# Ghostish/Open3DSOT

Hardware: AMD Instinct MI355X
Metric: template/search pairs/sec (fwd+bwd), BAT KITTI-Car 512/1024 pts (higher is better)
Workload: dtype f32; 1 GPU; BAT_Car.yaml KITTI-Car, template 512 / search 1024 pts, batch 48 per GPU, fwd+bwd+Adam, fp32; global_batch=48, parallelism=dp1, fused_kernels=True, hip_graph=True, rccl_world_size=1

## Files before the change

### open3dsot_amd/csrc/mlp_direct.hip

```cpp
#include <type_traits>
#include "mlp_common.hpp"

namespace {

constexpr int DT_M = 64;

template <int NT>
__device__ __forceinline__ void ldv(float (&d)[NT], const float* p) {
    if constexpr (NT == 4) {
        const float4 t = *reinterpret_cast<const float4*>(p);
        d[0] = t.x; d[1] = t.y; d[2] = t.z; d[3] = t.w;
    } else if constexpr (NT == 2) {
        const float2 t = *reinterpret_cast<const float2*>(p);
        d[0] = t.x; d[1] = t.y;
    } else {
        d[0] = *p;
    }
}
template <int NT>
__device__ __forceinline__ void stv(float* p, const float (&d)[NT]) {
    if constexpr (NT == 4)      *reinterpret_cast<float4*>(p) = make_float4(d[0], d[1], d[2], d[3]);
    else if constexpr (NT == 2) *reinterpret_cast<float2*>(p) = make_float2(d[0], d[1]);
    else                        *p = d[0];
}

template <int NT>
struct RawB {
    float v[4][NT];
    float y[4][NT];
    float4 c1, c2, c3;
};

enum BMode { B_PLAIN = 0, B_XFORM = 1, B_DY = 2, B_DYPOOL = 3 };

struct DirectArgs {
    const float* A;
    const float* X;
    const float* Y;
    const float* c1; const float* c2; const float* c3;
    const float2* pk; int ns;
    float* Out;
    int M, K, P, B;
    const float* w;
    const int32_t* meta;
    long start1;
    float* part;
    const float* stat_c;
    const float* Yprev; const float* scale_p; const float* shift_p; const float* mean_p;
    const float* bias;
    const float* resid;
    const float* cbias; int cb_N, cb_B;
    int tail_slots; long extra_row0;
};

template <int MODE, int NT>
__device__ __forceinline__ void load_b(const DirectArgs& a, const float* xb, const float* yb, long rowP, int kb,
                                       long pool_base, int np, RawB<NT>& f) {
#pragma unroll
    for (int s = 0; s < 4; ++s) {
        if (MODE != B_DYPOOL) ldv<NT>(f.v[s], xb + (long)(kb + s) * rowP);
        if (MODE >= B_DY) ldv<NT>(f.y[s], yb + (long)(kb + s) * rowP);
        if constexpr (MODE == B_DYPOOL && NT >= 2) {
            const float2 t = a.pk[pool_base + (long)(kb + s) * np];
            f.v[s][0] = t.x; f.v[s][1] = t.y;
        }
    }
    if (MODE != B_PLAIN) {
        f.c1 = *reinterpret_cast<const float4*>(a.c1 + kb);
        f.c2 = *reinterpret_cast<const float4*>(a.c2 + kb);
        if (MODE >= B_DY) f.c3 = *reinterpret_cast<const float4*>(a.c3 + kb);
    }
}

template <int MODE, int NT, int MT>
__device__ __forceinline__ void compute_group(const RawB<NT>& f, const float4& a0v, const float4& a1v, int kk,
                                              const float (&wv)[NT], f32x16 (&acc)[MT][NT]) {
    const float a0[4] = {a0v.x, a0v.y, a0v.z, a0v.w}, a1[4] = {a1v.x, a1v.y, a1v.z, a1v.w};
    const float c1[4] = {f.c1.x, f.c1.y, f.c1.z, f.c1.w}, c2[4] = {f.c2.x, f.c2.y, f.c2.z, f.c2.w};
    const float c3[4] = {f.c3.x, f.c3.y, f.c3.z, f.c3.w};
#pragma unroll
    for (int s = 0; s < 4; ++s) {
        float bv[NT];
        if constexpr (MODE == B_DYPOOL && NT >= 2) {
            const float go = f.v[s][0];
            const int ak = __float_as_int(f.v[s][1]);
#pragma unroll
            for (int t = 0; t < NT; ++t) bv[t] = (kk + t == ak) ? go : 0.f;
        } else {
#pragma unroll
            for (int t = 0; t < NT; ++t) bv[t] = f.v[s][t];
        }
        if (MODE == B_XFORM) {
#pragma unroll
            for (int t = 0; t < NT; ++t) bv[t] = fmaxf(fmaf(bv[t], c1[s], c2[s]), 0.f);
        } else if (MODE >= B_DY) {
#pragma unroll
            for (int t = 0; t < NT; ++t) bv[t] = fmaf(c1[s], bv[t], wv[t] * fmaf(c2[s], f.y[s][t], c3[s]));
        }
#pragma unroll
        for (int t = 0; t < NT; ++t) {
            acc[0][t] = mfma32(a0[s], bv[t], acc[0][t]);
            if constexpr (MT == 2) acc[1][t] = mfma32(a1[s], bv[t], acc[1][t]);
        }
    }
}

template <int WAVES, int MODE, int EPI, int NT, int MT = 2>
__device__ __forceinline__ void direct_gemm_body(DirectArgs& a, const int bx, const int by, const long part_row = -1) {
    constexpr int POS = 32 * NT;
    constexpr int DT_MW = 32 * MT;
    const int lane = threadIdx.x & 63, wave = threadIdx.x >> 6;
    const int l31 = lane & 31, h = lane >> 5;
    const int tiles_per_b = a.P / POS;
    const int tile = bx;
    const int b = tile / tiles_per_b, p0 = (tile - b * tiles_per_b) * POS;
    if (a.meta) {
        const long c0 = (long)tile * POS;
        const int seg = (a.start1 > 0 && c0 >= a.start1) ? 1 : 0;
        if (c0 - (seg ? a.start1 : 0) >= a.meta[4 * seg]) return;
        if (seg) {
            if (a.c1) a.c1 += a.K;
            if (a.c2) a.c2 += a.K;
            if (a.c3) a.c3 += a.K;
            if (a.stat_c) a.stat_c += a.M;
            if (a.scale_p) { a.scale_p += a.M; a.shift_p += a.M; a.mean_p += a.M; }
        }
    }
    const int m0 = (by * WAVES + wave) * DT_MW;
    const int p = p0 + NT * l31;
    float wv[NT];
#pragma unroll
    for (int t = 0; t < NT; ++t) wv[t] = 1.f;
    if (a.w) ldv<NT>(wv, a.w + (long)b * a.P + p);
    const long rowP = a.P;
    const float* xb = (MODE != B_DYPOOL) ? a.X + (long)b * a.K * rowP + p : nullptr;
    const float* yb = (MODE >= B_DY) ? a.Y + (long)b * a.K * rowP + p : nullptr;
    const float* wa = a.A + (long)(m0 + l31) * a.K + 4 * h;
    const long wstep = 32L * a.K;
    int np = 1, kk = 0;
    long pool_base = 0;
    if (MODE == B_DYPOOL) {
        np = a.P / a.ns;
        const int j = p / a.ns;
        kk = p - j * a.ns;
        pool_base = (long)b * a.K * np + j;
    }

    f32x16 acc[MT][NT];
#pragma unroll
    for (int i = 0; i < MT; ++i)
#pragma unroll
        for (int t = 0; t < NT; ++t)
#pragma unroll
            for (int r = 0; r < 16; ++r) acc[i][t][r] = 0.f;

    const int G = a.K / 8;
    RawB<NT> f[2];
    float4 wa0[2], wa1[2];
    auto load = [&](auto stc, int g) {
        constexpr int st = decltype(stc)::value;
        const int kb = 8 * g + 4 * h;
        load_b<MODE, NT>(a, xb, yb, rowP, kb, pool_base, np, f[st]);
        wa0[st] = *reinterpret_cast<const float4*>(wa + 8 * g);
        if constexpr (MT == 2) wa1[st] = *reinterpret_cast<const float4*>(wa + 8 * g + wstep);
        else wa1[st] = wa0[st];
    };
    {
        load(std::integral_constant<int, 0>{}, 0);
        for (int g = 0; g < G; g += 2) {
            load(std::integral_constant<int, 1>{}, g + 1);
            __builtin_amdgcn_sched_barrier(0);
            compute_group<MODE, NT, MT>(f[0], wa0[0], wa1[0], kk, wv, acc);
            __builtin_amdgcn_sched_barrier(0);
            load(std::integral_constant<int, 0>{}, g + 2 < G ? g + 2 : G - 1);
            __builtin_amdgcn_sched_barrier(0);
            compute_group<MODE, NT, MT>(f[1], wa0[1], wa1[1], kk, wv, acc);
            __builtin_amdgcn_sched_barrier(0);
        }
    }

    int cloud = 0;
    if constexpr (EPI == 3) cloud = (int)(((long)b * a.P + p0) / a.cb_N);
    const bool stats = EPI != 2 && a.part != nullptr;
    float4 kc1[MT][4], kc2[MT][4];
    if constexpr (EPI != 1) {
#pragma unroll
        for (int i = 0; i < MT; ++i)
#pragma unroll
            for (int q = 0; q < 4; ++q) {
                const int mb = m0 + 32 * i + 4 * h + 8 * q;
                kc1[i][q] = kc2[i][q] = make_float4(0.f, 0.f, 0.f, 0.f);
                if constexpr (EPI == 2) {
                    if (a.bias) kc1[i][q] = *reinterpret_cast<const float4*>(a.bias + mb);
                } else {
                    if (a.stat_c) kc1[i][q] = *reinterpret_cast<const float4*>(a.stat_c + mb);
                    if constexpr (EPI == 3) {
                        kc2[i][q].x = a.cbias[(long)(mb + 0) * a.cb_B + cloud];
                        kc2[i][q].y = a.cbias[(long)(mb + 1) * a.cb_B + cloud];
                        kc2[i][q].z = a.cbias[(long)(mb + 2) * a.cb_B + cloud];
                        kc2[i][q].w = a.cbias[(long)(mb + 3) * a.cb_B + cloud];
                    }
                }
            }
    }
#pragma unroll
    for (int i = 0; i < MT; ++i) {
        float red[32];
#pragma unroll
        for (int hb = 0; hb < 2; ++hb) {
            const int mb = m0 + 32 * i + 16 * hb + 4 * h;
            const long ob = ((long)b * a.M + mb) * rowP + p;
            float ex[8][NT];
            float4 k1[2], k2[2], k3[2];
            if constexpr (EPI == 1 || EPI == 2) {
                const float* src = EPI == 1 ? a.Yprev : a.resid;
#pragma unroll
                for (int r = 0; r < 8; ++r) {
#pragma unroll
                    for (int t = 0; t < NT; ++t) ex[r][t] = 0.f;
                    if (EPI == 1 || src) ldv<NT>(ex[r], src + ob + (long)(8 * (r >> 2) + (r & 3)) * rowP);
                }
            }
#pragma unroll
            for (int q = 0; q < 2; ++q) {
                k3[q] = make_float4(0.f, 0.f, 0.f, 0.f);
                if constexpr (EPI == 1) {
                    k1[q] = *reinterpret_cast<const float4*>(a.scale_p + mb + 8 * q);
                    k2[q] = *reinterpret_cast<const float4*>(a.shift_p + mb + 8 * q);
                    k3[q] = *reinterpret_cast<const float4*>(a.mean_p + mb + 8 * q);
                } else {
                    k1[q] = kc1[i][2 * hb + q];
                    k2[q] = kc2[i][2 * hb + q];
                }
            }
#pragma unroll
            for (int r8 = 0; r8 < 8; ++r8) {
                const int q = r8 >> 2, j = r8 & 3, r = 8 * hb + r8;
                const float c1 = j == 0 ? k1[q].x : j == 1 ? k1[q].y : j == 2 ? k1[q].z : k1[q].w;
                const float c2 = j == 0 ? k2[q].x : j == 1 ? k2[q].y : j == 2 ? k2[q].z : k2[q].w;
                const float c3 = j == 0 ? k3[q].x : j == 1 ? k3[q].y : j == 2 ? k3[q].z : k3[q].w;
                float v[NT];
#pragma unroll
                for (int t = 0; t < NT; ++t) v[t] = acc[i][t][r];
                float s1 = 0.f, s2 = 0.f;
                if constexpr (EPI == 1) {
#pragma unroll
                    for (int t = 0; t < NT; ++t) {
                        v[t] = fmaf(ex[r8][t], c1, c2) > 0.f ? v[t] : 0.f;
                        s1 += v[t];
                        s2 = fmaf(v[t], ex[r8][t] - c3, s2);
                    }
                } else if constexpr (EPI == 2) {
#pragma unroll
                    for (int t = 0; t < NT; ++t) v[t] = (v[t] + c1) + ex[r8][t];
                } else {
#pragma unroll
                    for (int t = 0; t < NT; ++t) {
                        if constexpr (EPI == 3) v[t] += c2;
                        s1 = fmaf(wv[t], v[t], s1);
                        s2 += wv[t] * (v[t] - c1) * (v[t] - c1);
                    }
                }
                stv<NT>(a.Out + ob + (long)(8 * q + j) * rowP, v);
                red[r] = s1;
                red[16 + r] = s2;
            }
        }
        if (stats) {
            reduce_scatter32(red, l31);
            a.part[(part_row >= 0 ? part_row : (long)tile) * 2 * a.M + (long)(l31 >> 4) * a.M + m0 + 32 * i + acc_row(l31 & 15, h)] = red[0];
        }
    }
}


template <int WAVES, int MODE, int EPI, int NT, int MT = 2>
__global__ __launch_bounds__(WAVES * 64) __attribute__((amdgpu_waves_per_eu(2, (NT == 4 && MT == 2) ? 2 : 4)))
void direct_gemm_kernel(DirectArgs a) {
    direct_gemm_body<WAVES, MODE, EPI, NT, MT>(a, blockIdx.x, blockIdx.y);
}

template <int WAVES, int MODE, int EPI>
__global__ __launch_bounds__(WAVES * 64) __attribute__((amdgpu_waves_per_eu(2, 2)))
void direct_gemm_tail_kernel(DirectArgs a) {
    const int tile = blockIdx.x;
    const int seg = (a.start1 > 0 && (long)tile * 128 >= a.start1) ? 1 : 0;
    const int t0 = seg ? (int)(a.start1 / 128) : 0;
    const int cap = a.start1 > 0 ? (seg ? (int)((a.P - a.start1) / 128) : (int)(a.start1 / 128)) : a.P / 128;
    const int T = a.meta[4 * seg] / 128;
    const TailPlan pl = tail_plan(T, a.tail_slots, cap);
    const int tl = tile - t0;
    if (tl < pl.full) { direct_gemm_body<WAVES, MODE, EPI, 4, 2>(a, tile, blockIdx.y); return; }
    const int u = tl - pl.full;
    if (u >= pl.R * pl.f) return;
    const int j = u / pl.f, blk = u - j * pl.f;
    const int tt = t0 + pl.full + j;
    const long row = blk == 0 ? (long)tt : a.extra_row0 + (long)seg * a.tail_slots + (long)j * (pl.f - 1) + (blk - 1);
    if (pl.f == 4) direct_gemm_body<WAVES, MODE, EPI, 1, 2>(a, tt * 4 + blk, blockIdx.y, row);
    else           direct_gemm_body<WAVES, MODE, EPI, 2, 2>(a, tt * 2 + blk, blockIdx.y, row);
}

template <int WAVES, int MODE, int EPI, int NT, int MT>
__global__ __launch_bounds__(WAVES * 64) __attribute__((amdgpu_waves_per_eu(2, NT == 4 ? 2 : 4)))
void direct_gemm_pair_kernel(DirectArgs a0, DirectArgs a1) {
    if (blockIdx.z == 0) {
        if ((int)blockIdx.y * WAVES * 32 * MT < a0.M) direct_gemm_body<WAVES, MODE, EPI, NT, MT>(a0, blockIdx.x, blockIdx.y);
    } else {
        if ((int)blockIdx.y * WAVES * 32 * MT < a1.M) direct_gemm_body<WAVES, MODE, EPI, NT, MT>(a1, blockIdx.x, blockIdx.y);
    }
}

constexpr int SK_ROWS = 32, SK_COLS = 64;

__device__ __forceinline__ float reduce_scatter8(float (&x)[8], int l31) {
#pragma unroll
    for (int m = 4; m >= 1; m >>= 1) {
        const bool up = (l31 & m) != 0;
#pragma unroll
        for (int v = 0; v < m; ++v) {
            float lo = x[v], hi = x[v + m];
            asm volatile("" : "+v"(lo), "+v"(hi));
            const float keep = up ? hi : lo;
            const float send = up ? lo : hi;
            x[v] = keep + __shfl_xor(send, m, 64);
        }
    }
    float r = x[0];
    r += __shfl_xor(r, 8, 64);
    r += __shfl_xor(r, 16, 64);
    return r;
}

template <int MODE, int EPI>
__device__ __forceinline__ void splitk_body(DirectArgs& a, const int bx, const int by, float* __restrict__ red) {
    static_assert(MODE <= B_DY && EPI <= 2, "split-K tile: plain / transformed / BatchNorm-backward operands only");
    constexpr int NT = 2;
    const int lane = threadIdx.x & 63, wave = threadIdx.x >> 6;
    const int l31 = lane & 31, h = lane >> 5;
    const int tiles_per_b = a.P / SK_COLS;
    const int tile = bx;
    const int b = tile / tiles_per_b, p0 = (tile - b * tiles_per_b) * SK_COLS;
    if (a.meta) {
        const long c0 = (long)tile * SK_COLS;
        const int seg = (a.start1 > 0 && c0 >= a.start1) ? 1 : 0;
        if (c0 - (seg ? a.start1 : 0) >= a.meta[4 * seg]) return;
        if (seg) {
            if (a.c1) a.c1 += a.K;
            if (a.c2) a.c2 += a.K;
            if (a.c3) a.c3 += a.K;
            if (a.stat_c) a.stat_c += a.M;
            if (a.scale_p) { a.scale_p += a.M; a.shift_p += a.M; a.mean_p += a.M; }
        }
    }
    const int m0 = by * SK_ROWS;
    const int p = p0 + NT * l31;
    float wv[NT] = {1.f, 1.f};
    if (a.w) ldv<NT>(wv, a.w + (long)b * a.P + p);
    const long rowP = a.P;
    const float* xb = a.X + (long)b * a.K * rowP + p;
    const float* yb = (MODE >= B_DY) ? a.Y + (long)b * a.K * rowP + p : nullptr;
    const float* wa = a.A + (long)(m0 + l31) * a.K + 4 * h;

    const int mrow = m0 + 8 * wave + 4 * h;
    const long ob = ((long)b * a.M + mrow) * rowP + p;
    float ex[4][NT];
    float4 k1 = make_float4(0.f, 0.f, 0.f, 0.f), k2 = k1, k3 = k1;
    if constexpr (EPI == 1 || EPI == 2) {
        const float* src = EPI == 1 ? a.Yprev : a.resid;
#pragma unroll
        for (int j = 0; j < 4; ++j) {
            ex[j][0] = ex[j][1] = 0.f;
            if (EPI == 1 || src) ldv<NT>(ex[j], src + ob + (long)j * rowP);
        }
    }
    if constexpr (EPI == 1) {
        k1 = *reinterpret_cast<const float4*>(a.scale_p + mrow);
        k2 = *reinterpret_cast<const float4*>(a.shift_p + mrow);
        k3 = *reinterpret_cast<const float4*>(a.mean_p + mrow);
    } else if constexpr (EPI == 2) {
        if (a.bias) k1 = *reinterpret_cast<const float4*>(a.bias + mrow);
    } else {
        if (a.stat_c) k1 = *reinterpret_cast<const float4*>(a.stat_c + mrow);
    }

    f32x16 acc[1][NT];
#pragma unroll
    for (int t = 0; t < NT; ++t)
#pragma unroll
        for (int r = 0; r < 16; ++r) acc[0][t][r] = 0.f;

    const int npair = a.K / 16;
    const int q = npair / 4, rem = npair - 4 * q;
    const int ps = wave * q + (wave < rem ? wave : rem);
    const int gs = 2 * ps, ge = 2 * (ps + q + (wave < rem ? 1 : 0));
    RawB<NT> f[2];
    float4 wa0[2];
    auto load = [&](auto stc, int g) {
        constexpr int st = decltype(stc)::value;
        load_b<MODE, NT>(a, xb, yb, rowP, 8 * g + 4 * h, 0, 1, f[st]);
        wa0[st] = *reinterpret_cast<const float4*>(wa + 8 * g);
    };
    if (gs < ge) {
        load(std::integral_constant<int, 0>{}, gs);
        for (int g = gs; g < ge; g += 2) {
            load(std::integral_constant<int, 1>{}, g + 1);
            __builtin_amdgcn_sched_barrier(0);
            compute_group<MODE, NT, 1>(f[0], wa0[0], wa0[0], 0, wv, acc);
            __builtin_amdgcn_sched_barrier(0);
            load(std::integral_constant<int, 0>{}, g + 2 < ge ? g + 2 : ge - 1);
            __builtin_amdgcn_sched_barrier(0);
            compute_group<MODE, NT, 1>(f[1], wa0[1], wa0[1], 0, wv, acc);
            __builtin_amdgcn_sched_barrier(0);
        }
    }

#pragma unroll
    for (int r = 0; r < 16; ++r)
        *reinterpret_cast<float2*>(red + ((wave * SK_ROWS + acc_row(r, h)) * SK_COLS + NT * l31)) =
            make_float2(acc[0][0][r], acc[0][1][r]);
    __syncthreads();
    float x8[8];
    const bool stats = EPI != 2 && a.part != nullptr;
#pragma unroll
    for (int j = 0; j < 4; ++j) {
        const int row = 8 * wave + 4 * h + j;
        float v[NT] = {0.f, 0.f};
#pragma unroll
        for (int w4 = 0; w4 < 4; ++w4) {
            const float2 t = *reinterpret_cast<const float2*>(red + ((w4 * SK_ROWS + row) * SK_COLS + NT * l31));
            v[0] += t.x; v[1] += t.y;
        }
        const float c1 = j == 0 ? k1.x : j == 1 ? k1.y : j == 2 ? k1.z : k1.w;
        const float c2 = j == 0 ? k2.x : j == 1 ? k2.y : j == 2 ? k2.z : k2.w;
        const float c3 = j == 0 ? k3.x : j == 1 ? k3.y : j == 2 ? k3.z : k3.w;
        float s1 = 0.f, s2 = 0.f;
        if constexpr (EPI == 1) {
#pragma unroll
            for (int t = 0; t < NT; ++t) {
                v[t] = fmaf(ex[j][t], c1, c2) > 0.f ? v[t] : 0.f;
                s1 += v[t];
                s2 = fmaf(v[t], ex[j][t] - c3, s2);
            }
        } else if constexpr (EPI == 2) {
#pragma unroll
            for (int t = 0; t < NT; ++t) v[t] = (v[t] + c1) + ex[j][t];
        } else {
#pragma unroll
            for (int t = 0; t < NT; ++t) {
                s1 = fmaf(wv[t], v[t], s1);
                s2 += wv[t] * (v[t] - c1) * (v[t] - c1);
            }
        }
        stv<NT>(a.Out + ob + (long)j * rowP, v);
        x8[j] = s1;
        x8[4 + j] = s2;
    }
    if (stats) {
        const float r = reduce_scatter8(x8, l31);
        if (l31 < 8) a.part[(long)tile * 2 * a.M + (long)(l31 >> 2) * a.M + mrow + (l31 & 3)] = r;
    }
}

template <int MODE, int EPI>
__global__ __launch_bounds__(256) __attribute__((amdgpu_waves_per_eu(3, 4)))
void splitk_gemm_kernel(DirectArgs a) {
    __shared__ float red[4 * SK_ROWS * SK_COLS];
    splitk_body<MODE, EPI>(a, blockIdx.x, blockIdx.y, red);
}

template <int MODE, int EPI>
__global__ __launch_bounds__(256) __attribute__((amdgpu_waves_per_eu(3, 4)))
void splitk_gemm_pair_kernel(DirectArgs a0, DirectArgs a1) {
    __shared__ float red[4 * SK_ROWS * SK_COLS];
    if (blockIdx.z == 0) {
        if ((int)blockIdx.y * SK_ROWS < a0.M) splitk_body<MODE, EPI>(a0, blockIdx.x, blockIdx.y, red);
    } else {
        if ((int)blockIdx.y * SK_ROWS < a1.M) splitk_body<MODE, EPI>(a1, blockIdx.x, blockIdx.y, red);
    }
}

static long splitk_max() { return 16L << 20; }
static bool splitk_ok(const DirectArgs& a, int tile) {
    return tile == 64 && a.K % 16 == 0 && a.K >= 64 && a.M % SK_ROWS == 0 && a.P % SK_COLS == 0 && !a.pk &&
           (long)a.M * a.B * a.P <= splitk_max();
}
template <int MODE, int EPI>
int launch_splitk(const DirectArgs& a, hipStream_t st) {
    if constexpr (MODE <= B_DY && EPI <= 2) {
        hipLaunchKernelGGL((splitk_gemm_kernel<MODE, EPI>), dim3(a.B * (a.P / SK_COLS), a.M / SK_ROWS), dim3(256), 0, st, a);
        return o3d_launch_status();
    } else {
        return O3D_EINVAL;
    }
}

template <int MODE, int EPI, int NT, int MT = 2>
int launch_direct_nt(const DirectArgs& a, hipStream_t st) {
    const int tiles = a.B * (a.P / (32 * NT));
    const int slabs = a.M / (32 * MT);
    if constexpr (NT == 4 && MT == 2 && MODE != B_DYPOOL && EPI <= 1) {
        if (a.tail_slots > 0 && a.meta && a.B == 1) {
            if (slabs % 4 == 0)      hipLaunchKernelGGL((direct_gemm_tail_kernel<4, MODE, EPI>), dim3(tiles, slabs / 4), dim3(256), 0, st, a);
            else if (slabs % 2 == 0) hipLaunchKernelGGL((direct_gemm_tail_kernel<2, MODE, EPI>), dim3(tiles, slabs / 2), dim3(128), 0, st, a);
            else                     hipLaunchKernelGGL((direct_gemm_tail_kernel<1, MODE, EPI>), dim3(tiles, slabs), dim3(64), 0, st, a);
            return o3d_launch_status();
        }
    }
    if (slabs % 4 == 0) {
        hipLaunchKernelGGL((direct_gemm_kernel<4, MODE, EPI, NT, MT>), dim3(tiles, slabs / 4), dim3(256), 0, st, a);
    } else if (slabs % 2 == 0) {
        hipLaunchKernelGGL((direct_gemm_kernel<2, MODE, EPI, NT, MT>), dim3(tiles, slabs / 2), dim3(128), 0, st, a);
    } else {
        hipLaunchKernelGGL((direct_gemm_kernel<1, MODE, EPI, NT, MT>), dim3(tiles, slabs), dim3(64), 0, st, a);
    }
    return o3d_launch_status();
}

static int pw_tile(long P, int M) { return o3d_direct_tile(P, M, 0); }

template <int MODE, int EPI>
int launch_direct_small(const DirectArgs& a, int tile, hipStream_t st) {
    if constexpr (MODE <= B_DY && EPI <= 2) {
        if (splitk_ok(a, tile)) return launch_splitk<MODE, EPI>(a, st);
    }
    if constexpr (MODE != B_DYPOOL) {
        if (tile == 128 && a.M <= 128) return launch_direct_nt<MODE, EPI, 4, 1>(a, st);
    }
    return tile == 64 ? launch_direct_nt<MODE, EPI, 2>(a, st) : launch_direct_nt<MODE, EPI, 4>(a, st);
}

template <int MODE, int EPI>
int launch_direct(const DirectArgs& a, int tile, hipStream_t st) {
    if constexpr (MODE <= B_DY && EPI <= 2) {
        if (splitk_ok(a, tile)) return launch_splitk<MODE, EPI>(a, st);
    }
    return tile == 64 ? launch_direct_nt<MODE, EPI, 2>(a, st) : launch_direct_nt<MODE, EPI, 4>(a, st);
}

}

bool o3d_direct_ok(int M, int K, int P) { return M % DT_M == 0 && K % 16 == 0 && P % 128 == 0; }

static int g_tail_override = -1;
extern "C" int o3d_direct_tail_override(int slots) { g_tail_override = slots; return O3D_OK; }

extern "C" int o3d_direct_tail_slots(int M) {
    if (g_tail_override >= 0) return (M > 0 && M % DT_M == 0) ? g_tail_override : 0;
    static int cus_of[64] = {};
    int dev = 0;
    if (hipGetDevice(&dev) != hipSuccess || dev < 0 || dev >= 64) dev = 0;
    if (cus_of[dev] == 0) {
        int n = 0;
        if (hipDeviceGetAttribute(&n, hipDeviceAttributeMultiprocessorCount, dev) != hipSuccess || n <= 0) n = 256;
        cus_of[dev] = n;
    }
    const int cus = cus_of[dev];
    if (M <= 0 || M % DT_M != 0) return 0;
    const int slabs = M / DT_M;
    const int waves = slabs % 4 == 0 ? 4 : (slabs % 2 == 0 ? 2 : 1);
    const int per_tile = slabs / waves;
    const int slots = (8 / waves) * cus / per_tile;
    return slots >= 64 ? slots : 0;
}

extern "C" int o3d_direct_tile(long P, int M, int compact) {
    (void)M; (void)compact;
    return P <= 65536L ? 64 : 128;
}

int o3d_direct_fwd(const float* X, const float* W, const float* in_scale, const float* in_shift, int B, int Cin,
                   int Cout, int P, float* Y, float* part, const float* stat_c, const float* w, const int32_t* meta,
                   long start1, int tile, hipStream_t st) {
    DirectArgs a = {};
    a.w = w; a.meta = meta; a.start1 = start1;
    a.A = W; a.X = X; a.c1 = in_scale; a.c2 = in_shift; a.Out = Y; a.M = Cout; a.K = Cin; a.P = P; a.B = B;
    a.part = part; a.stat_c = stat_c; a.ns = 4;
    if (meta && tile == 128 && B == 1 && in_scale) { a.tail_slots = o3d_direct_tail_slots(Cout); a.extra_row0 = P / 128; }
    return in_scale ? launch_direct<B_XFORM, 0>(a, tile, st) : launch_direct<B_PLAIN, 0>(a, tile, st);
}

int o3d_direct_dgrad(const float* dN, const float* pk, int ns,
                     const float* Y, const float* A1, const float* A2, const float* A3, const float* Wt, int B,
                     int Cin, int Cout, int P, const float* Yprev, const float* scale_p, const float* shift_p,
                     const float* mean_p, float* dNprev, float* part, const float* w, const int32_t* meta,
                     long start1, int tile, hipStream_t st) {
    DirectArgs a = {};
    a.w = w; a.meta = meta; a.start1 = start1;
    a.A = Wt; a.X = dN; a.Y = Y; a.c1 = A1; a.c2 = A2; a.c3 = A3; a.pk = reinterpret_cast<const float2*>(pk); a.ns = ns;
    a.Out = dNprev; a.M = Cin; a.K = Cout; a.P = P; a.B = B; a.part = part;
    a.Yprev = Yprev; a.scale_p = scale_p; a.shift_p = shift_p; a.mean_p = mean_p;
    if (meta && tile == 128 && B == 1 && dN) { a.tail_slots = o3d_direct_tail_slots(Cin); a.extra_row0 = P / 128; }
    if (dN && !Y) { a.c1 = a.c2 = a.c3 = nullptr; return launch_direct<B_PLAIN, 1>(a, tile, st); }
    return dN ? launch_direct<B_DY, 1>(a, tile, st) : launch_direct<B_DYPOOL, 1>(a, tile, st);
}


extern "C" int o3d_pw_tile(long P, int M) { return pw_tile(P, M); }

extern "C" int o3d_pw_fwd(const float* X, const float* W, const float* in_scale, const float* in_shift,
                          const float* bias, const float* resid, int Cin, int Cout, long P, float* Y, float* part,
                          const float* stat_c, void* stream) {
    if (!X || !W || !Y || P <= 0 || P > 0x7fffffff || P % 64 != 0 || Cin <= 0 || Cin % 16 != 0 || Cout <= 0 ||
        Cout % DT_M != 0 || (in_scale == nullptr) != (in_shift == nullptr) || (part && (bias || resid)))
        return O3D_EINVAL;
    const int tile = pw_tile(P, Cout);
    if (tile == 128 && P % 128 != 0) return O3D_EINVAL;
    DirectArgs a = {};
    a.A = W; a.X = X; a.c1 = in_scale; a.c2 = in_shift; a.Out = Y; a.M = Cout; a.K = Cin; a.P = (int)P; a.B = 1;
    a.part = part; a.stat_c = stat_c; a.ns = 4; a.bias = bias; a.resid = resid;
    hipStream_t st = reinterpret_cast<hipStream_t>(stream);
    if (part || (!bias && !resid))
        return in_scale ? launch_direct_small<B_XFORM, 0>(a, tile, st) : launch_direct_small<B_PLAIN, 0>(a, tile, st);
    return in_scale ? launch_direct_small<B_XFORM, 2>(a, tile, st) : launch_direct_small<B_PLAIN, 2>(a, tile, st);
}

extern "C" int o3d_pw_dgrad(const float* dN, const float* Y, const float* A1, const float* A2, const float* A3,
                            const float* Wt, int Cin, int Cout, long P, const float* Yprev, const float* scale_p,
                            const float* shift_p, const float* mean_p, const float* resid, float* dNprev, float* part,
                            void* stream) {
    if (!dN || !Wt || !dNprev || P <= 0 || P > 0x7fffffff || P % 64 != 0 || Cin <= 0 || Cin % DT_M != 0 ||
        Cout <= 0 || Cout % 16 != 0 || (Y && (!A1 || !A2 || !A3)) ||
        (Yprev && (!scale_p || !shift_p || !mean_p || !part || resid)) || (!Yprev && part))
        return O3D_EINVAL;
    const int tile = pw_tile(P, Cin);
    if (tile == 128 && P % 128 != 0) return O3D_EINVAL;
    DirectArgs a = {};
    a.A = Wt; a.X = dN; a.Y = Y; a.c1 = A1; a.c2 = A2; a.c3 = A3; a.ns = 4;
    a.Out = dNprev; a.M = Cin; a.K = Cout; a.P = (int)P; a.B = 1; a.part = part;
    a.Yprev = Yprev; a.scale_p = scale_p; a.shift_p = shift_p; a.mean_p = mean_p; a.resid = resid;
    hipStream_t st = reinterpret_cast<hipStream_t>(stream);
    if (Yprev) return Y ? launch_direct_small<B_DY, 1>(a, tile, st) : launch_direct_small<B_PLAIN, 1>(a, tile, st);
    return Y ? launch_direct_small<B_DY, 2>(a, tile, st) : launch_direct_small<B_PLAIN, 2>(a, tile, st);
}

namespace {
template <int MODE, int EPI, int NT, int MT>
int launch_pair_nt(const DirectArgs& a, const DirectArgs& b, hipStream_t st) {
    const int tiles = a.P / (32 * NT);
    const int sa = a.M / (32 * MT), sb = b.M / (32 * MT);
    const int smax = sa > sb ? sa : sb;
    if (sa % 4 == 0 && sb % 4 == 0)
        hipLaunchKernelGGL((direct_gemm_pair_kernel<4, MODE, EPI, NT, MT>), dim3(tiles, smax / 4, 2), dim3(256), 0, st, a, b);
    else if (sa % 2 == 0 && sb % 2 == 0)
        hipLaunchKernelGGL((direct_gemm_pair_kernel<2, MODE, EPI, NT, MT>), dim3(tiles, smax / 2, 2), dim3(128), 0, st, a, b);
    else
        hipLaunchKernelGGL((direct_gemm_pair_kernel<1, MODE, EPI, NT, MT>), dim3(tiles, smax, 2), dim3(64), 0, st, a, b);
    return o3d_launch_status();
}

static int small_class(const DirectArgs& a, int tile) {
    if (splitk_ok(a, tile)) return 4;
    return tile == 64 ? 2 : 3;
}

template <int MODE, int EPI>
int launch_pair(const DirectArgs& a, const DirectArgs& b, int cls, hipStream_t st) {
    if (cls == 4) {
        const int sa = a.M / SK_ROWS, sb = b.M / SK_ROWS;
        hipLaunchKernelGGL((splitk_gemm_pair_kernel<MODE, EPI>), dim3(a.P / SK_COLS, sa > sb ? sa : sb, 2), dim3(256), 0, st, a, b);
        return o3d_launch_status();
    }
    return cls == 2 ? launch_pair_nt<MODE, EPI, 2, 2>(a, b, st) : launch_pair_nt<MODE, EPI, 4, 2>(a, b, st);
}

static bool pw_fwd_args_ok(const o3d_pw_fwd_args& q) {
    return q.X && q.W && q.Y && q.P > 0 && q.P <= 0x7fffffff && q.P % 64 == 0 && q.Cin > 0 && q.Cin % 16 == 0 && q.Cout > 0 &&
           q.Cout % DT_M == 0 && (q.in_scale == nullptr) == (q.in_shift == nullptr) && !(q.part && (q.bias || q.resid));
}
static DirectArgs pw_fwd_direct(const o3d_pw_fwd_args& q) {
    DirectArgs a = {};
    a.A = q.W; a.X = q.X; a.c1 = q.in_scale; a.c2 = q.in_shift; a.Out = q.Y; a.M = q.Cout; a.K = q.Cin; a.P = (int)q.P; a.B = 1;
    a.part = q.part; a.stat_c = q.stat_c; a.ns = 4; a.bias = q.bias; a.resid = q.resid;
    return a;
}
static bool pw_dgrad_args_ok(const o3d_pw_dgrad_args& q) {
    return q.dN && q.Wt && q.dNprev && q.P > 0 && q.P <= 0x7fffffff && q.P % 64 == 0 && q.Cin > 0 && q.Cin % DT_M == 0 &&
           q.Cout > 0 && q.Cout % 16 == 0 && !(q.Y && (!q.A1 || !q.A2 || !q.A3)) &&
           !(q.Yprev && (!q.scale_p || !q.shift_p || !q.mean_p || !q.part || q.resid)) && !(!q.Yprev && q.part);
}
static DirectArgs pw_dgrad_direct(const o3d_pw_dgrad_args& q) {
    DirectArgs a = {};
    a.A = q.Wt; a.X = q.dN; a.Y = q.Y; a.c1 = q.A1; a.c2 = q.A2; a.c3 = q.A3; a.ns = 4;
    a.Out = q.dNprev; a.M = q.Cin; a.K = q.Cout; a.P = (int)q.P; a.B = 1; a.part = q.part;
    a.Yprev = q.Yprev; a.scale_p = q.scale_p; a.shift_p = q.shift_p; a.mean_p = q.mean_p; a.resid = q.resid;
    return a;
}
}

extern "C" int o3d_pw_fwd_pair(const o3d_pw_fwd_args* pa, const o3d_pw_fwd_args* pb, void* stream) {
    if (!pa || !pb || !pw_fwd_args_ok(*pa) || !pw_fwd_args_ok(*pb)) return O3D_EINVAL;
    const o3d_pw_fwd_args &x = *pa, &y = *pb;
    const int ta = pw_tile(x.P, x.Cout), tb = pw_tile(y.P, y.Cout);
    if ((ta == 128 && x.P % 128) || (tb == 128 && y.P % 128)) return O3D_EINVAL;
    DirectArgs a = pw_fwd_direct(x), b = pw_fwd_direct(y);
    const bool epi2a = !(x.part || (!x.bias && !x.resid)), epi2b = !(y.part || (!y.bias && !y.resid));
    const int ca = small_class(a, ta), cb = small_class(b, tb);
    hipStream_t st = reinterpret_cast<hipStream_t>(stream);
    if (x.P != y.P || ta != tb || ca != cb || epi2a != epi2b || (x.in_scale == nullptr) != (y.in_scale == nullptr)) {
        const int rc = o3d_pw_fwd(x.X, x.W, x.in_scale, x.in_shift, x.bias, x.resid, x.Cin, x.Cout, x.P, x.Y, x.part, x.stat_c, stream);
        if (rc != O3D_OK) return rc;
        return o3d_pw_fwd(y.X, y.W, y.in_scale, y.in_shift, y.bias, y.resid, y.Cin, y.Cout, y.P, y.Y, y.part, y.stat_c, stream);
    }
    if (!epi2a) return x.in_scale ? launch_pair<B_XFORM, 0>(a, b, ca, st) : launch_pair<B_PLAIN, 0>(a, b, ca, st);
    return x.in_scale ? launch_pair<B_XFORM, 2>(a, b, ca, st) : launch_pair<B_PLAIN, 2>(a, b, ca, st);
}

extern "C" int o3d_pw_dgrad_pair(const o3d_pw_dgrad_args* pa, const o3d_pw_dgrad_args* pb, void* stream) {
    if (!pa || !pb || !pw_dgrad_args_ok(*pa) || !pw_dgrad_args_ok(*pb)) return O3D_EINVAL;
    const o3d_pw_dgrad_args &x = *pa, &y = *pb;
    const int ta = pw_tile(x.P, x.Cin), tb = pw_tile(y.P, y.Cin);
    if ((ta == 128 && x.P % 128) || (tb == 128 && y.P % 128)) return O3D_EINVAL;
    DirectArgs a = pw_dgrad_direct(x), b = pw_dgrad_direct(y);
    const int ca = small_class(a, ta), cb = small_class(b, tb);
    hipStream_t st = reinterpret_cast<hipStream_t>(stream);
    if (x.P != y.P || ta != tb || ca != cb || (x.Yprev == nullptr) != (y.Yprev == nullptr) || (x.Y == nullptr) != (y.Y == nullptr)) {
        const int rc = o3d_pw_dgrad(x.dN, x.Y, x.A1, x.A2, x.A3, x.Wt, x.Cin, x.Cout, x.P, x.Yprev, x.scale_p, x.shift_p, x.mean_p,
                                    x.resid, x.dNprev, x.part, stream);
        if (rc != O3D_OK) return rc;
        return o3d_pw_dgrad(y.dN, y.Y, y.A1, y.A2, y.A3, y.Wt, y.Cin, y.Cout, y.P, y.Yprev, y.scale_p, y.shift_p, y.mean_p, y.resid,
                            y.dNprev, y.part, stream);
    }
    if (x.Yprev) return x.Y ? launch_pair<B_DY, 1>(a, b, ca, st) : launch_pair<B_PLAIN, 1>(a, b, ca, st);
    return x.Y ? launch_pair<B_DY, 2>(a, b, ca, st) : launch_pair<B_PLAIN, 2>(a, b, ca, st);
}

extern "C" int o3d_pw_fwd_cloud(const float* X, const float* W, const float* cbias, int B, int N, int Cin, int Cout,
                                float* Y, float* part, const float* stat_c, void* stream) {
    const long P = (long)B * N;
    if (!X || !W || !cbias || !Y || B <= 0 || N <= 0 || N % 128 != 0 || P > 0x7fffffff || Cin <= 0 || Cin % 16 != 0 ||
        Cout <= 0 || Cout % DT_M != 0)
        return O3D_EINVAL;
    DirectArgs a = {};
    a.A = W; a.X = X; a.Out = Y; a.M = Cout; a.K = Cin; a.P = (int)P; a.B = 1; a.part = part; a.stat_c = stat_c; a.ns = 4;
    a.cbias = cbias; a.cb_N = N; a.cb_B = B;
    return launch_direct_nt<B_PLAIN, 3, 4>(a, reinterpret_cast<hipStream_t>(stream));
}
```

Before: 9032 pairs/s.

## Stage epilogue residual and per-K constants into LDS via async global-to-LDS DMA

```diff
diff --git a/open3dsot_amd/csrc/mlp_direct.hip b/open3dsot_amd/csrc/mlp_direct.hip
--- a/open3dsot_amd/csrc/mlp_direct.hip
+++ b/open3dsot_amd/csrc/mlp_direct.hip
@@ -30,6 +30,31 @@
     float y[4][NT];
     float4 c1, c2, c3;
 };
+
+__device__ __forceinline__ void glds16(const float* src, unsigned lds_dst, bool on = true) {
+    unsigned keep;
+    lds_dst = __builtin_amdgcn_readfirstlane(lds_dst);
+    const int go = __builtin_amdgcn_readfirstlane((int)on);
+    asm volatile("s_cmp_lg_u32 %3, 0\n\ts_cbranch_scc0 .Lglds_skip%=\n\t"
+                 "s_mov_b32 %0, m0\n\ts_mov_b32 m0, %2\n\ts_nop 0\n\tglobal_load_lds_dwordx4 %1, off\n\ts_mov_b32 m0, %0\n"
+                 ".Lglds_skip%=:"
+                 : "=&s"(keep) : "v"(src), "s"(lds_dst), "s"(go) : "memory", "scc");
+}
+__device__ __forceinline__ void glds16x3_wait(const float* s0, const float* s1, const float* s2, unsigned lds_dst, bool on) {
+    unsigned keep;
+    lds_dst = __builtin_amdgcn_readfirstlane(lds_dst);
+    const int go = __builtin_amdgcn_readfirstlane((int)on);
+    asm volatile("s_cmp_lg_u32 %5, 0\n\ts_cbranch_scc0 .Lglds3_skip%=\n\t"
+                 "s_mov_b32 %0, m0\n\ts_mov_b32 m0, %4\n\ts_nop 0\n\tglobal_load_lds_dwordx4 %1, off\n\t"
+                 "s_add_u32 m0, m0, 0x400\n\ts_nop 0\n\tglobal_load_lds_dwordx4 %2, off\n\t"
+                 "s_add_u32 m0, m0, 0x400\n\ts_nop 0\n\tglobal_load_lds_dwordx4 %3, off\n\t"
+                 "s_mov_b32 m0, %0\n\ts_waitcnt vmcnt(0)\n"
+                 ".Lglds3_skip%=:"
+                 : "=&s"(keep) : "v"(s0), "v"(s1), "v"(s2), "s"(lds_dst), "s"(go) : "memory", "scc");
+}
+template <int N>
+__device__ __forceinline__ void stage_wait_vm() { asm volatile("s_waitcnt vmcnt(%0)" :: "i"(N) : "memory"); }
+__device__ __forceinline__ void stage_wait_lds() { asm volatile("s_waitcnt lgkmcnt(0)" ::: "memory"); }
 
 enum BMode { B_PLAIN = 0, B_XFORM = 1, B_DY = 2, B_DYPOOL = 3 };
 
@@ -53,7 +78,7 @@
     int tail_slots; long extra_row0;
 };
 
-template <int MODE, int NT>
+template <int MODE, int NT, bool KLDS = false>
 __device__ __forceinline__ void load_b(const DirectArgs& a, const float* xb, const float* yb, long rowP, int kb,
                                        long pool_base, int np, RawB<NT>& f) {
 #pragma unroll
@@ -65,7 +90,7 @@
             f.v[s][0] = t.x; f.v[s][1] = t.y;
         }
     }
-    if (MODE != B_PLAIN) {
+    if (MODE != B_PLAIN && !KLDS) {
         f.c1 = *reinterpret_cast<const float4*>(a.c1 + kb);
         f.c2 = *reinterpret_cast<const float4*>(a.c2 + kb);
         if (MODE >= B_DY) f.c3 = *reinterpret_cast<const float4*>(a.c3 + kb);
@@ -73,11 +98,12 @@
 }
 
 template <int MODE, int NT, int MT>
-__device__ __forceinline__ void compute_group(const RawB<NT>& f, const float4& a0v, const float4& a1v, int kk,
+__device__ __forceinline__ void compute_group(const RawB<NT>& f, const float4& c1v, const float4& c2v, const float4& c3v,
+                                              const float4& a0v, const float4& a1v, int kk,
                                               const float (&wv)[NT], f32x16 (&acc)[MT][NT]) {
     const float a0[4] = {a0v.x, a0v.y, a0v.z, a0v.w}, a1[4] = {a1v.x, a1v.y, a1v.z, a1v.w};
-    const float c1[4] = {f.c1.x, f.c1.y, f.c1.z, f.c1.w}, c2[4] = {f.c2.x, f.c2.y, f.c2.z, f.c2.w};
-    const float c3[4] = {f.c3.x, f.c3.y, f.c3.z, f.c3.w};
+    const float c1[4] = {c1v.x, c1v.y, c1v.z, c1v.w}, c2[4] = {c2v.x, c2v.y, c2v.z, c2v.w};
+    const float c3[4] = {c3v.x, c3v.y, c3v.z, c3v.w};
 #pragma unroll
     for (int s = 0; s < 4; ++s) {
         float bv[NT];
@@ -105,9 +131,18 @@
     }
 }
 
+constexpr int STAGE_ROWC = 768, STAGE_KCHUNK = 256;
+template <int NT, int MODE> constexpr int stage_wave_bytes() { return 4096 * NT + STAGE_ROWC + (MODE >= B_DY ? 3 * 4 * STAGE_KCHUNK : 0); }
+template <int EPI, int MT> constexpr bool staged_epilogue() { return EPI == 1 && MT == 2; }
+
 template <int WAVES, int MODE, int EPI, int NT, int MT = 2>
-__device__ __forceinline__ void direct_gemm_body(DirectArgs& a, const int bx, const int by, const long part_row = -1) {
+__device__ __forceinline__ void direct_gemm_body(DirectArgs& a, const int bx, const int by, const long part_row = -1,
+                                                 char* stage = nullptr) {
     constexpr int POS = 32 * NT;
+    constexpr bool STAGE = staged_epilogue<EPI, MT>();
+    constexpr int ND = 4 * NT;
+    constexpr int LP = 4 / NT;
+    constexpr bool KLDS = STAGE && MODE >= B_DY;
     constexpr int DT_MW = 32 * MT;
     const int lane = threadIdx.x & 63, wave = threadIdx.x >> 6;
     const int l31 = lane & 31, h = lane >> 5;
@@ -146,6 +181,36 @@
         pool_base = (long)b * a.K * np + j;
     }
 
+    const float* ysrc = nullptr;
+    unsigned stage_dst = 0;
+    const char* stage_rd = nullptr;
+    if constexpr (STAGE) {
+        ysrc = a.Yprev + ((long)b * a.M + m0 + 4 * h) * rowP + p0 + NT * (l31 & ~(LP - 1));
+        stage_dst = __builtin_amdgcn_readfirstlane((unsigned)(uintptr_t)stage + wave * stage_wave_bytes<NT, MODE>());
+        stage_rd = stage + wave * stage_wave_bytes<NT, MODE>() + 16 * (32 * h + (l31 & ~(LP - 1))) + 4 * NT * (l31 & (LP - 1));
+    }
+    auto dma = [&](int i, int d, bool on = true) __attribute__((always_inline)) {
+        const int rr = LP * d + (l31 & (LP - 1));
+        glds16(ysrc + (long)(32 * i + (rr & 3) + 8 * (rr >> 2)) * rowP, stage_dst + 1024u * d, on);
+    };
+    auto stage_off = [&](int r) __attribute__((always_inline)) { return 1024 * (r / LP) + 16 * (r & (LP - 1)); };
+    auto dma_consts = [&]() __attribute__((always_inline)) {
+        const float *sp = a.scale_p, *hp = a.shift_p, *mp = a.mean_p;
+        const float* kp = (lane < 16 ? sp : lane < 32 ? hp : mp) + m0 + 4 * (lane & 15);
+        if (lane < 48) glds16(kp, stage_dst + 4096u * NT);
+    };
+    auto dma_kconsts = [&](int k0, bool on) __attribute__((always_inline)) {
+        const int kq = min(k0 + 4 * lane, a.K - 4);
+        glds16x3_wait(a.c1 + kq, a.c2 + kq, a.c3 + kq, stage_dst + 4096u * NT + STAGE_ROWC, on);
+    };
+    float4 pk1 = make_float4(0.f, 0.f, 0.f, 0.f), pk2 = pk1, pk3 = pk1;
+    auto read_kconsts = [&](int g) __attribute__((always_inline)) {
+        const char* kb = stage + wave * stage_wave_bytes<NT, MODE>() + 4096 * NT + STAGE_ROWC + 4 * ((8 * g + 4 * h) & (STAGE_KCHUNK - 1));
+        pk1 = *reinterpret_cast<const float4*>(kb);
+        pk2 = *reinterpret_cast<const float4*>(kb + 1024);
+        pk3 = *reinterpret_cast<const float4*>(kb + 2048);
+    };
+
     f32x16 acc[MT][NT];
 #pragma unroll
     for (int i = 0; i < MT; ++i)
@@ -160,22 +225,41 @@
     auto load = [&](auto stc, int g) {
         constexpr int st = decltype(stc)::value;
         const int kb = 8 * g + 4 * h;
-        load_b<MODE, NT>(a, xb, yb, rowP, kb, pool_base, np, f[st]);
+        load_b<MODE, NT, KLDS>(a, xb, yb, rowP, kb, pool_base, np, f[st]);
         wa0[st] = *reinterpret_cast<const float4*>(wa + 8 * g);
         if constexpr (MT == 2) wa1[st] = *reinterpret_cast<const float4*>(wa + 8 * g + wstep);
         else wa1[st] = wa0[st];
     };
+    int nd = 0;
     {
         load(std::integral_constant<int, 0>{}, 0);
+        if constexpr (STAGE) {
+            dma_consts();
+            for (; nd + G < ND; ++nd) dma(0, nd);
+        }
+        if constexpr (KLDS) {
+            dma_kconsts(0, true);
+            read_kconsts(0);
+        }
         for (int g = 0; g < G; g += 2) {
             load(std::integral_constant<int, 1>{}, g + 1);
+            if constexpr (STAGE) { dma(0, nd, nd < ND); ++nd; }
             __builtin_amdgcn_sched_barrier(0);
-            compute_group<MODE, NT, MT>(f[0], wa0[0], wa1[0], kk, wv, acc);
+            if constexpr (KLDS) compute_group<MODE, NT, MT>(f[0], pk1, pk2, pk3, wa0[0], wa1[0], kk, wv, acc);
+            else                compute_group<MODE, NT, MT>(f[0], f[0].c1, f[0].c2, f[0].c3, wa0[0], wa1[0], kk, wv, acc);
             __builtin_amdgcn_sched_barrier(0);
             load(std::integral_constant<int, 0>{}, g + 2 < G ? g + 2 : G - 1);
+            if constexpr (STAGE) { dma(0, nd, nd < ND); ++nd; }
+            if constexpr (KLDS) read_kconsts(g + 1);
             __builtin_amdgcn_sched_barrier(0);
-            compute_group<MODE, NT, MT>(f[1], wa0[1], wa1[1], kk, wv, acc);
+            if constexpr (KLDS) compute_group<MODE, NT, MT>(f[1], pk1, pk2, pk3, wa0[1], wa1[1], kk, wv, acc);
+            else                compute_group<MODE, NT, MT>(f[1], f[1].c1, f[1].c2, f[1].c3, wa0[1], wa1[1], kk, wv, acc);
             __builtin_amdgcn_sched_barrier(0);
+            if constexpr (KLDS) {
+                const int gn = g + 2 < G ? g + 2 : G - 1;
+                dma_kconsts(8 * gn, gn % (STAGE_KCHUNK / 8) == 0);
+                read_kconsts(gn);
+            }
         }
     }
 
@@ -212,7 +296,8 @@
             const long ob = ((long)b * a.M + mb) * rowP + p;
             float ex[8][NT];
             float4 k1[2], k2[2], k3[2];
-            if constexpr (EPI == 1 || EPI == 2) {
+            if constexpr (STAGE) {
+            } else if constexpr (EPI == 1 || EPI == 2) {
                 const float* src = EPI == 1 ? a.Yprev : a.resid;
 #pragma unroll
                 for (int r = 0; r < 8; ++r) {
@@ -224,7 +309,8 @@
 #pragma unroll
             for (int q = 0; q < 2; ++q) {
                 k3[q] = make_float4(0.f, 0.f, 0.f, 0.f);
-                if constexpr (EPI == 1) {
+                if constexpr (STAGE) {
+                } else if constexpr (EPI == 1) {
                     k1[q] = *reinterpret_cast<const float4*>(a.scale_p + mb + 8 * q);
                     k2[q] = *reinterpret_cast<const float4*>(a.shift_p + mb + 8 * q);
                     k3[q] = *reinterpret_cast<const float4*>(a.mean_p + mb + 8 * q);
@@ -236,6 +322,29 @@
 #pragma unroll
             for (int r8 = 0; r8 < 8; ++r8) {
                 const int q = r8 >> 2, j = r8 & 3, r = 8 * hb + r8;
+                if constexpr (STAGE) if (j == 0) {
+                    const int c = 2 * hb + q;
+                    if (i == 0 && c == 0) stage_wait_vm<0>();
+                    if (i == 1 && c == 0) stage_wait_vm<16 + 3 * (ND / 4)>();
+                    if (i == 1 && c == 1) stage_wait_vm<16 + 2 * (ND / 4)>();
+                    if (i == 1 && c == 2) stage_wait_vm<16 + 1 * (ND / 4)>();
+                    if (i == 1 && c == 3) stage_wait_vm<16>();
+#pragma unroll
+                    for (int jj = 0; jj < 4; ++jj)
+                        ldv<NT>(ex[4 * q + jj], reinterpret_cast<const float*>(stage_rd + stage_off(4 * c + jj)));
+                    const char* kb = stage + wave * stage_wave_bytes<NT, MODE>() + 4096 * NT + 16 * (8 * i + 2 * c + h);
+                    k1[q] = *reinterpret_cast<const float4*>(kb);
+                    k2[q] = *reinterpret_cast<const float4*>(kb + 256);
+                    k3[q] = *reinterpret_cast<const float4*>(kb + 512);
+                    if (i == 0) {
+                        stage_wait_lds();
+#pragma unroll
+                        for (int d = 0; d < ND / 4; ++d) {
+                            dma(1, c * (ND / 4) + d);
+                            __builtin_amdgcn_sched_barrier(0);
+                        }
+                    }
+                }
                 const float c1 = j == 0 ? k1[q].x : j == 1 ? k1[q].y : j == 2 ? k1[q].z : k1[q].w;
                 const float c2 = j == 0 ? k2[q].x : j == 1 ? k2[q].y : j == 2 ? k2[q].z : k2[q].w;
                 const float c3 = j == 0 ? k3[q].x : j == 1 ? k3[q].y : j == 2 ? k3[q].z : k3[q].w;
@@ -277,12 +386,22 @@
 template <int WAVES, int MODE, int EPI, int NT, int MT = 2>
 __global__ __launch_bounds__(WAVES * 64) __attribute__((amdgpu_waves_per_eu(2, (NT == 4 && MT == 2) ? 2 : 4)))
 void direct_gemm_kernel(DirectArgs a) {
-    direct_gemm_body<WAVES, MODE, EPI, NT, MT>(a, blockIdx.x, blockIdx.y);
+    if constexpr (staged_epilogue<EPI, MT>()) {
+        __shared__ float4 stage[WAVES * stage_wave_bytes<NT, MODE>() / 16];
+        direct_gemm_body<WAVES, MODE, EPI, NT, MT>(a, blockIdx.x, blockIdx.y, -1, reinterpret_cast<char*>(stage));
+    } else {
+        direct_gemm_body<WAVES, MODE, EPI, NT, MT>(a, blockIdx.x, blockIdx.y);
+    }
 }
 
 template <int WAVES, int MODE, int EPI>
 __global__ __launch_bounds__(WAVES * 64) __attribute__((amdgpu_waves_per_eu(2, 2)))
 void direct_gemm_tail_kernel(DirectArgs a) {
+    char* stage = nullptr;
+    if constexpr (staged_epilogue<EPI, 2>()) {
+        __shared__ float4 stage4[WAVES * stage_wave_bytes<4, MODE>() / 16];
+        stage = reinterpret_cast<char*>(stage4);
+    }
     const int tile = blockIdx.x;
     const int seg = (a.start1 > 0 && (long)tile * 128 >= a.start1) ? 1 : 0;
     const int t0 = seg ? (int)(a.start1 / 128) : 0;
@@ -290,23 +409,28 @@
     const int T = a.meta[4 * seg] / 128;
     const TailPlan pl = tail_plan(T, a.tail_slots, cap);
     const int tl = tile - t0;
-    if (tl < pl.full) { direct_gemm_body<WAVES, MODE, EPI, 4, 2>(a, tile, blockIdx.y); return; }
+    if (tl < pl.full) { direct_gemm_body<WAVES, MODE, EPI, 4, 2>(a, tile, blockIdx.y, -1, stage); return; }
     const int u = tl - pl.full;
     if (u >= pl.R * pl.f) return;
     const int j = u / pl.f, blk = u - j * pl.f;
     const int tt = t0 + pl.full + j;
     const long row = blk == 0 ? (long)tt : a.extra_row0 + (long)seg * a.tail_slots + (long)j * (pl.f - 1) + (blk - 1);
-    if (pl.f == 4) direct_gemm_body<WAVES, MODE, EPI, 1, 2>(a, tt * 4 + blk, blockIdx.y, row);
-    else           direct_gemm_body<WAVES, MODE, EPI, 2, 2>(a, tt * 2 + blk, blockIdx.y, row);
+    if (pl.f == 4) direct_gemm_body<WAVES, MODE, EPI, 1, 2>(a, tt * 4 + blk, blockIdx.y, row, stage);
+    else           direct_gemm_body<WAVES, MODE, EPI, 2, 2>(a, tt * 2 + blk, blockIdx.y, row, stage);
 }
 
 template <int WAVES, int MODE, int EPI, int NT, int MT>
 __global__ __launch_bounds__(WAVES * 64) __attribute__((amdgpu_waves_per_eu(2, NT == 4 ? 2 : 4)))
 void direct_gemm_pair_kernel(DirectArgs a0, DirectArgs a1) {
+    char* stage = nullptr;
+    if constexpr (staged_epilogue<EPI, MT>()) {
+        __shared__ float4 stage4[WAVES * stage_wave_bytes<NT, MODE>() / 16];
+        stage = reinterpret_cast<char*>(stage4);
+    }
     if (blockIdx.z == 0) {
-        if ((int)blockIdx.y * WAVES * 32 * MT < a0.M) direct_gemm_body<WAVES, MODE, EPI, NT, MT>(a0, blockIdx.x, blockIdx.y);
+        if ((int)blockIdx.y * WAVES * 32 * MT < a0.M) direct_gemm_body<WAVES, MODE, EPI, NT, MT>(a0, blockIdx.x, blockIdx.y, -1, stage);
     } else {
-        if ((int)blockIdx.y * WAVES * 32 * MT < a1.M) direct_gemm_body<WAVES, MODE, EPI, NT, MT>(a1, blockIdx.x, blockIdx.y);
+        if ((int)blockIdx.y * WAVES * 32 * MT < a1.M) direct_gemm_body<WAVES, MODE, EPI, NT, MT>(a1, blockIdx.x, blockIdx.y, -1, stage);
     }
 }
 
@@ -405,11 +529,11 @@
         for (int g = gs; g < ge; g += 2) {
             load(std::integral_constant<int, 1>{}, g + 1);
             __builtin_amdgcn_sched_barrier(0);
-            compute_group<MODE, NT, 1>(f[0], wa0[0], wa0[0], 0, wv, acc);
+            compute_group<MODE, NT, 1>(f[0], f[0].c1, f[0].c2, f[0].c3, wa0[0], wa0[0], 0, wv, acc);
             __builtin_amdgcn_sched_barrier(0);
             load(std::integral_constant<int, 0>{}, g + 2 < ge ? g + 2 : ge - 1);
             __builtin_amdgcn_sched_barrier(0);
-            compute_group<MODE, NT, 1>(f[1], wa0[1], wa0[1], 0, wv, acc);
+            compute_group<MODE, NT, 1>(f[1], f[1].c1, f[1].c2, f[1].c3, wa0[1], wa0[1], 0, wv, acc);
             __builtin_amdgcn_sched_barrier(0);
         }
     }
```

Result: no change. 9102 pairs/s, median of 6 (+0.8%).
